# cyu0330/ptbxl-multimodal

Hardware: AMD Instinct MI355X
Metric: ECG windows/s (train step) at 12x1000, batch 256 (higher is better)
Workload: dtype f32; 1 GPU; ECGCNN(5) train step fwd+BCE+bwd+AdamW, 12x1000, fp32, batch 256/GPU, global batch 256; global_batch=256, parallelism=dp1, loop=train_one_epoch, optimizer=FlatAdamW, priming_steps=30

## Files before the change

include/ecg_hip.h:

```cpp
#ifndef ECG_HIP_H
#define ECG_HIP_H

#include <stddef.h>
#include <stdint.h>

#ifdef __cplusplus
extern "C" {
#endif

typedef void *ecg_stream_t;

enum {
    ECG_OK = 0,
    ECG_EINVAL = 1,
    ECG_ELAUNCH = 2,
    ECG_ENODEV = 3
};

int ecg_version(void);
const char *ecg_last_error(void);
int ecg_check_device(void);


int ecg_conv1d_pack_weights(const float *w, float *w_fwd, float *w_bwd,
// ... 6 lines not shown
int ecg_pack_weights_grouped_mixed(const float *const *w, float *const *w_fwd, float *const *w_bwd,
                                   void *const *wb_fwd, void *const *wb_bwd, const int *C_out,
                                   const int *C_in, const int *K, int count, ecg_stream_t stream);

int ecg_conv1d_fwd_stat_partials(int N, int C_in, int C_out, int L, int K, int pad);

int ecg_conv1d_fwd(const float *x, const float *w_fwd, const float *bias, float *y,
                   float *stat_partials, int N, int C_in, int C_out, int L, int K, int pad,
                   ecg_stream_t stream);

int ecg_conv1d_bwd_data(const float *dy, const float *w_bwd, float *dx,
                        int N, int C_in, int C_out, int L, int K, int pad, ecg_stream_t stream);

int ecg_conv1d_dy_row_stride(int N, int C_in, int C_out, int L, int K, int pad, int need_dx);

int ecg_conv1d_multiplies_per_output_pair(int op, int C_in, int C_out, int K, int pad);
int ecg_conv1d_bwd_data_ld(const float *dy, int ldy, const float *w_bwd, float *dx,
                           int N, int C_in, int C_out, int L, int K, int pad, ecg_stream_t stream);
int ecg_conv1d_bwd_weight_bias_ld(const float *dy, int ldy, const float *x, float *dw, float *db,
                                  float *ws, int N, int C_in, int C_out, int L, int K, int pad,
                                  ecg_stream_t stream);

size_t ecg_conv1d_bwd_weight_ws_floats(int N, int C_in, int C_out, int L, int K, int pad);
int ecg_conv1d_bwd_weight_bias(const float *dy, const float *x, float *dw, float *db, float *ws,
                               int N, int C_in, int C_out, int L, int K, int pad,
                               ecg_stream_t stream);

int ecg_conv1d_bf16_supported(int C_in, int C_out, int K, int pad);
size_t ecg_conv1d_bf16_packed_elems(int C_reduce, int C_result, int K);
int ecg_conv1d_pack_weights_bf16(const float *w, void *wb_fwd, void *wb_bwd, int C_out, int C_in,
                                 int K, ecg_stream_t stream);
int ecg_conv1d_fwd_bf16_yh(const void *x, int x_bf16, int ldx, const void *wb_fwd, const float *bias, void *y_bf16,
                           int ldy, float *stat_partials, int N, int C_in, int C_out, int L, int K, int pad,
                           ecg_stream_t stream);
int ecg_conv1d_fwd_bf16_yh_stat_partials(int N, int C_in, int C_out, int L, int K, int pad, int x_bf16, int ldx, int ldy);
int ecg_conv1d_bf16_ring_tile(int N, int C_red, int C_res, int L_out, int K, int pad, int ld_in, int ld_out);
int ecg_bn_stats_relu_pool_fwd_h(const float *stat_partials, int P, long long count, float *running_mean,
                                 float *running_var, long long *num_batches_tracked, float momentum, float eps,
                                 const void *y_bf16, int ldy, const float *gamma, const float *beta, float *mean,
                                 float *invstd, void *p_bf16, int ldp, int N, int C, int L, ecg_stream_t stream);
int ecg_bn_stats_relu_pool_gap_fwd_yh(const float *stat_partials, int P, long long count, float *running_mean,
                                      float *running_var, long long *num_batches_tracked, float momentum, float eps,
                                      const void *y_bf16, int ldy, const float *gamma, const float *beta, float *mean,
                                      float *invstd, float *out, int N, int C, int L, ecg_stream_t stream);
int ecg_bn_relu_pool_bwd_h(const void *y_bf16, int ldyy, const void *dp, int dp_kind, int ldp, const float *gamma,
                           const float *beta, const float *mean, const float *invstd, void *dy_bf16, int ldy,
// ... 159 lines not shown
```

ptbxl-multimodal_amd/csrc/conv1d_api.hip:

```cpp
#include "common.h"

namespace ecg {
int direct_fwd_stat_partials(int N, int Lo);
int direct_fwd(const float *x, const float *wp, const float *bias, float *y, float *partials,
               int N, int Cin, int Cout, int L, int K, int pad, hipStream_t st);
size_t direct_wgrad_ws_floats(int N, int Cin, int Cout, int K);
int direct_wgrad(const float *dy, const float *x, float *dw, float *db, float *ws, int N, int Cin,
                 int Cout, int L, int K, int pad, hipStream_t st);
int pack_weights(const float *w, float *w_fwd, float *w_bwd, int Co, int Ci, int K,
                 hipStream_t st);
int pack_weights_grouped(const float *const *w, float *const *w_fwd, float *const *w_bwd, void *const *wb_fwd,
                         void *const *wb_bwd, const int *Co, const int *Ci, const int *K, int count, hipStream_t st);
bool mfma_fwd_supported(int Cin, int Cout, int K, int pad);
int mfma_fwd_stat_partials(int N, int Cin, int Cout, int Lo);
int mfma_fwd(const float *x, int ldx, const float *wp, const float *bias, float *y, float *partials,
             int N, int Cin, int Cout, int L, int K, int pad, hipStream_t st);
int mfma_fwd_eval_pool(const float *x, const float *wp, const float *bias, const float *gamma,
                       const float *beta, const float *mean, const float *var, float eps, float *p,
                       int N, int Cin, int Cout, int L, int K, int pad, hipStream_t st, int gap);
bool mfma_fwd_eval_gap_supported(int Cin, int Cout, int L, int K, int pad);
bool mfma_wgrad_supported(int Cin, int Cout, int K, int pad);
size_t mfma_wgrad_ws_floats(int N, int Cin, int Cout, int L, int K, int pad);
bool mfma_wgrad_dma_supported(int Cin, int Cout, int K);
int mfma_multiplies_per_pair(int op, int Cin, int Cout, int K, int pad);
int mfma_wgrad(const float *dy, int ldy, const float *x, float *dw, float *db, float *ws, int N,
               int Cin, int Cout, int L, int K, int pad, hipStream_t st);

static int check_conv_shape(int N, int Cin, int Cout, int L, int K, int pad) {
    ECG_REQUIRE(N > 0 && Cin > 0 && Cout > 0 && L > 0, "conv1d: N=%d C_in=%d C_out=%d L=%d must be > 0",
                N, Cin, Cout, L);
    ECG_REQUIRE(K >= 1 && K <= 31, "conv1d: kernel size %d outside [1,31]", K);
    ECG_REQUIRE(pad >= 0 && pad < K, "conv1d: padding %d outside [0,K)", pad);
    ECG_REQUIRE(L + 2 * pad - K + 1 > 0, "conv1d: empty output (L=%d K=%d pad=%d)", L, K, pad);
    ECG_REQUIRE(N <= 65535, "conv1d: N=%d exceeds grid.z limit 65535", N);
    return ECG_OK;
}
}

using namespace ecg;

ECG_API int ecg_conv1d_pack_weights(const float *w, float *w_fwd, float *w_bwd, int C_out,
                                    int C_in, int K, ecg_stream_t stream) {
    ECG_REQUIRE(w && (w_fwd || w_bwd), "pack_weights: null pointer");
    ECG_REQUIRE(C_out > 0 && C_in > 0 && K >= 1 && K <= 31, "pack_weights: bad shape");
    return pack_weights(w, w_fwd, w_bwd, C_out, C_in, K, as_stream(stream));
// ... 63 lines not shown
                                   int C_in, int C_out, int L, int K, int pad, ecg_stream_t stream) {
    int rc = check_conv_shape(N, C_in, C_out, L, K, pad);
    if (rc) return rc;
    ECG_REQUIRE(dy && w_bwd && dx, "conv1d_bwd_data: null pointer");
    const int Lo = L + 2 * pad - K + 1, padb = K - 1 - pad;
    ECG_REQUIRE(ldy >= Lo, "conv1d_bwd_data: dY row stride %d < row length %d", ldy, Lo);
    if (mfma_fwd_supported(C_out, C_in, K, padb))
        return mfma_fwd(dy, ldy, w_bwd, nullptr, dx, nullptr, N, C_out, C_in, Lo, K, padb, as_stream(stream));
    ECG_REQUIRE(ldy == Lo, "conv1d_bwd_data: this shape needs dense dY rows (stride %d != %d); "
                "use the stride ecg_conv1d_dy_row_stride returns", ldy, Lo);
    return direct_fwd(dy, w_bwd, nullptr, dx, nullptr, N, C_out, C_in, Lo, K, padb, as_stream(stream));
}

ECG_API int ecg_conv1d_bwd_data(const float *dy, const float *w_bwd, float *dx, int N, int C_in,
                                int C_out, int L, int K, int pad, ecg_stream_t stream) {
    return ecg_conv1d_bwd_data_ld(dy, L + 2 * pad - K + 1, w_bwd, dx, N, C_in, C_out, L, K, pad, stream);
}

ECG_API size_t ecg_conv1d_bwd_weight_ws_floats(int N, int C_in, int C_out, int L, int K, int pad) {
    if (mfma_wgrad_supported(C_in, C_out, K, pad)) return mfma_wgrad_ws_floats(N, C_in, C_out, L, K, pad);
    return direct_wgrad_ws_floats(N, C_in, C_out, K);
}

ECG_API int ecg_conv1d_bwd_weight_bias_ld(const float *dy, int ldy, const float *x, float *dw,
                                          float *db, float *ws, int N, int C_in, int C_out, int L,
                                          int K, int pad, ecg_stream_t stream) {
    int rc = check_conv_shape(N, C_in, C_out, L, K, pad);
    if (rc) return rc;
    ECG_REQUIRE(dy && x && dw && ws, "conv1d_bwd_weight_bias: null pointer");
    const int Lo = L + 2 * pad - K + 1;
    ECG_REQUIRE(ldy >= Lo, "conv1d_bwd_weight_bias: dY row stride %d < row length %d", ldy, Lo);
    if (mfma_wgrad_supported(C_in, C_out, K, pad))
        return mfma_wgrad(dy, ldy, x, dw, db, ws, N, C_in, C_out, L, K, pad, as_stream(stream));
    ECG_REQUIRE(ldy == Lo, "conv1d_bwd_weight_bias: this shape needs dense dY rows (stride %d != %d); "
                "use the stride ecg_conv1d_dy_row_stride returns", ldy, Lo);
    return direct_wgrad(dy, x, dw, db, ws, N, C_in, C_out, L, K, pad, as_stream(stream));
}

ECG_API int ecg_conv1d_bwd_weight_bias(const float *dy, const float *x, float *dw, float *db,
                                       float *ws, int N, int C_in, int C_out, int L, int K, int pad,
                                       ecg_stream_t stream) {
    return ecg_conv1d_bwd_weight_bias_ld(dy, L + 2 * pad - K + 1, x, dw, db, ws, N, C_in, C_out, L, K,
                                         pad, stream);
}

ECG_API int ecg_conv1d_bn_relu_pool_eval_supported(int C_in, int C_out, int K, int pad) {
// ... 42 lines not shown
```

ptbxl-multimodal_amd/csrc/conv1d_mfma.hip:

```cpp
#include "common.h"
#include <cstdlib>
#include <type_traits>

namespace ecg {

typedef float f32x16 __attribute__((ext_vector_type(16)));
typedef float f32x4 __attribute__((ext_vector_type(4)));

constexpr int kKM = 15;

#ifdef ECG_STAMP
__device__ unsigned long long *g_stamps = nullptr;
#define ECG_STAMP_AT(slot) do { if (g_stamps && threadIdx.x == 0) { \
    g_stamps[(size_t)blockIdx.x * 8 + (slot)] = __builtin_amdgcn_s_memtime(); \
    if ((slot) == 0) g_stamps[(size_t)blockIdx.x * 8 + 7] = __builtin_amdgcn_s_memrealtime(); \
    if ((slot) == 4) g_stamps[(size_t)blockIdx.x * 8 + 6] = __builtin_amdgcn_s_memrealtime(); } } while (0)
#else
#define ECG_STAMP_AT(slot) do { } while (0)
#endif

__device__ __forceinline__ f32x16 mfma32(float a, float b, f32x16 c) {
    return __builtin_amdgcn_mfma_f32_32x32x2f32(a, b, c, 0, 0, 0);
}

__device__ __forceinline__ void glds16(const void *base_in, unsigned voff, unsigned dst) {
    const unsigned long long b = (unsigned long long)base_in;
    const unsigned blo = (unsigned)__builtin_amdgcn_readfirstlane((int)(unsigned)b);
    const unsigned bhi = (unsigned)__builtin_amdgcn_readfirstlane((int)(unsigned)(b >> 32));
    const void *base = (const void *)(((unsigned long long)bhi << 32) | blo);
    unsigned keep;
    asm volatile("s_mov_b32 %0, m0\n\ts_mov_b32 m0, %3\n\ts_nop 0\n\tglobal_load_lds_dwordx4 %1, %2\n\ts_mov_b32 m0, %0"
                 : "=&s"(keep) : "v"(voff), "s"(base), "s"(dst) : "memory");
}

__device__ __forceinline__ void wait_lgkm_f(int n) {
    switch (n) {
        case 1: __builtin_amdgcn_s_waitcnt(0xC17F); break;
        case 2: __builtin_amdgcn_s_waitcnt(0xC27F); break;
        case 3: __builtin_amdgcn_s_waitcnt(0xC37F); break;
        case 4: __builtin_amdgcn_s_waitcnt(0xC47F); break;
        default: break;
    }
}

__device__ __forceinline__ int acc_row(int r, int half) { return (r & 3) + 8 * (r >> 2) + 4 * half; }

enum { EPI_PLAIN = 0, EPI_STATS = 1, EPI_EVAL = 2, EPI_EVAL_GAP = 3 };
#ifndef ECG_FWD_FL
#define ECG_FWD_FL 1
#endif

__device__ __forceinline__ int xcd_chunked(int bid, int nwg) {
    const int q = nwg >> 3, r = nwg & 7, xcd = bid & 7;
    return (xcd < r ? xcd * (q + 1) : r * (q + 1) + (xcd - r) * q) + (bid >> 3);
}
struct EvalEpi { const float *gamma, *beta, *mean, *var; float eps; int gap; };

template <int CO_T, int T_T, int WCO, int WT, int EPI>
__global__ __launch_bounds__(256, 2) void conv1d_mfma_fwd_kernel(
    const float *__restrict__ x, const float *__restrict__ wp, const float *__restrict__ bias,
    float *__restrict__ y, float *__restrict__ partials, int Cin, int Cout, int L, int ldx, int Lo,
    int pad, int P, int tiles_t, EvalEpi ev) {
    constexpr bool STATS = (EPI == EPI_STATS), GAP = (EPI == EPI_EVAL_GAP);
    static_assert(WCO * WT == 4, "4 waves per workgroup");
    constexpr int KK = kKM, CI_C = 4, NST = KK * CI_C / 2;
    constexpr int MC = CO_T / WCO / 32, MT = T_T / WT / 32;
    static_assert(MC >= 1 && MT >= 1, "wave tile must hold at least one 32x32 accumulator");
    constexpr int XS = T_T + 16;
    constexpr int WSZ = KK * CI_C * CO_T;
    constexpr int NDMA = (WSZ + 255) / 256;
    constexpr int WPAD = NDMA * 256;
    constexpr int DPW = (NDMA + 3) / 4;
    constexpr int XEL = CI_C * XS;
    constexpr int XLOADS = (XEL + 255) / 256;
    constexpr int IMG = WPAD + XEL;
    constexpr int REDF = (STATS || GAP) ? 4 * (CO_T / WCO) * 2 : 0;
    static_assert(REDF <= IMG, "stat scratch aliases image 0");
    static_assert(NST >= 2 + DPW + XLOADS, "not enough steps to spread the staging over");
// ... 861 lines not shown
    static_assert(NST % 4 == 0, "whole groups of four steps");
    constexpr int XSPAN = T_T + KK - 1;
    constexpr int XS = ((XSPAN - KK + 31) / 32) * 32 + KK;
    constexpr int NCI = (R_T + KK - 2) / KK + 1;
    constexpr int XEL = NCI * XS, XLOADS = (XEL + 255) / 256;
    constexpr int AEL = M_T * T_T;
    constexpr int NDMA = AEL / 256;
    constexpr int DPW = NDMA / 4;
    constexpr int IMG = ((AEL + XEL + 63) / 64) * 64;
    constexpr int ACCF = MC * MR * 16 * 64;
    static_assert(WK == 1 || WM * WR * ACCF + 4 * 32 <= 2 * IMG, "accumulator exchange must fit the dead images");
    static_assert(XS >= XSPAN, "x row stride too small");
    static_assert(NDMA % 4 == 0, "dY image must split evenly over the four waves");
    static_assert(XLOADS <= 32, "mask bits");
    static_assert(NST >= 2 * XLOADS + DPW, "not enough steps to spread the staging over");

    __shared__ __attribute__((aligned(1024))) float lds[2 * IMG];
    ECG_STAMP_AT(0);

    const int tid = threadIdx.x, lane = tid & 63, wave = tid >> 6;
    const int half = lane >> 5, l31 = lane & 31;
    const int R = Cin * KK;
    const int RT = (R + R_T - 1) / R_T, CT = Cout / M_T;
    const int tile = xcd_chunked(blockIdx.x, gridDim.x);
    const int tile_r = tile % RT, tile_cs = tile / RT;
    const int r0 = tile_r * R_T, co0 = (tile_cs % CT) * M_T, s = tile_cs / CT;
    const int wk = wave % WK, wr = (wave / WK) % WR, wm = wave / (WK * WR);
    const int wm0 = wm * (M_T / WM), wr0 = wr * (R_T / WR), wt0 = wk * TW;
    const int ci_base = r0 / KK;
    const int ntt = (Lo + T_T - 1) / T_T;
    const int it_begin = (int)((long long)N * ntt * s / S), it_end = (int)((long long)N * ntt * (s + 1) / S);

    int xcol[MR];
#pragma unroll
    for (int j = 0; j < MR; ++j) {
        int r = r0 + wr0 + 32 * j + l31;
        if (r >= R) r = R - 1;
        const int ci = r / KK;
        xcol[j] = (ci - ci_base) * XS + (r - ci * KK);
    }

    f32x16 acc[MC][MR], acc2[MC][MR];
    f32x16 zero16;
#pragma unroll
    for (int r = 0; r < 16; ++r) zero16[r] = 0.f;
#pragma unroll
    for (int a = 0; a < MC; ++a)
#pragma unroll
        for (int b = 0; b < MR; ++b) { acc[a][b] = zero16; acc2[a][b] = zero16; }
    float bsum[MC], bsum2[MC];
#pragma unroll
    for (int a = 0; a < MC; ++a) bsum[a] = bsum2[a] = 0.f;
    const bool want_bias = (tile_r == 0) && (wr == 0);

// ... 187 lines not shown
    asm volatile("s_waitcnt vmcnt(0)" ::: "memory");
#endif
    ECG_STAMP_AT(4);
}

template <int M_T, int R_T, int WM, int WR, int FL, int T_T>
__global__ __launch_bounds__(256, 2) void conv1d_mfma_wgrad_ffa_kernel(
    const float *__restrict__ dy, const float *__restrict__ x, float *__restrict__ slab, int N,
    int Cin, int Cout, int L, int Lo, int ldy, int pad, int S) {
    static_assert(WM * WR == 4, "4 waves per workgroup");
    static_assert(kKM == 15, "tap split 8 + 7");
    static_assert(T_T == 64 || T_T == 128, "64 or 128 time steps per stage");
    constexpr int LPR = T_T / 4, RPP = 64 / LPR;
    constexpr int MC = M_T / WM / 32, MR = R_T / WR / 32;
    constexpr int NST = T_T / 4, NGRP = NST / 4;
    constexpr int XS = T_T + 16;
    static_assert(XS % 64 == 16, "x rows 16 banks apart");
    constexpr int NCI = (R_T + 6) / 7 + 1;
    constexpr int XEL = NCI * XS, XLOADS = (XEL + 255) / 256;
    constexpr int AEL = M_T * T_T;
    constexpr int NDMA = AEL / 256;
    constexpr int DPW = NDMA / 4;
    constexpr int IMG = ((AEL + XEL + 63) / 64) * 64;
    constexpr int OPS = 2 * XLOADS + DPW;
    static_assert(NDMA % 4 == 0, "dY image must split evenly over the four waves");
    static_assert(XLOADS <= 32, "mask bits");
    static_assert(2 * IMG * 4 <= 80 * 1024, "two workgroups per CU");

    __shared__ __attribute__((aligned(1024))) float lds[2 * IMG];
    ECG_STAMP_AT(0);

    const int tid = threadIdx.x, lane = tid & 63, wave = tid >> 6;
    const int half = lane >> 5, l31 = lane & 31;
    const int RU = Cin * 8, RV = Cin * 7;
    const int TU = (RU + R_T - 1) / R_T, TV = (RV + R_T - 1) / R_T;
    const int RT = 2 * TU + TV, CT = Cout / M_T;
    const int tile = xcd_chunked(blockIdx.x, gridDim.x);
    const int tile_r = tile % RT, tile_cs = tile / RT;
    const int fam = tile_r < TU ? 0 : (tile_r < TU + TV ? 1 : 2);
    const int tile_rf = tile_r - (fam == 0 ? 0 : (fam == 1 ? TU : TU + TV));
    const int NJ = fam == 1 ? 7 : 8, RF = Cin * NJ, offf = fam == 0 ? 0 : (fam == 1 ? RU : RU + RV);
    const int r0 = tile_rf * R_T, co0 = (tile_cs % CT) * M_T, s = tile_cs / CT;
    const int wr = wave % WR, wm = wave / WR;
    const int wm0 = wm * (M_T / WM), wr0 = wr * (R_T / WR);
    const int ci_base = r0 / NJ;
    const int ntt = (Lo + T_T - 1) / T_T;
    const int it_begin = (int)((long long)N * ntt * s / S), it_end = (int)((long long)N * ntt * (s + 1) / S);

    int xcol[MR];
#pragma unroll
    for (int j = 0; j < MR; ++j) {
        int r = r0 + wr0 + 32 * j + l31;
        if (r >= RF) r = RF - 1;
        const int ci = r / NJ;
        xcol[j] = (ci - ci_base) * XS + 2 * (r - ci * NJ) + 8 * half;
    }

    f32x16 acc[MC][MR], acc2[MC][MR];
    f32x16 zero16;
#pragma unroll
    for (int r = 0; r < 16; ++r) zero16[r] = 0.f;
#pragma unroll
    for (int a = 0; a < MC; ++a)
#pragma unroll
        for (int b = 0; b < MR; ++b) { acc[a][b] = zero16; acc2[a][b] = zero16; }
    float bsum[MC], bsum2[MC];
#pragma unroll
    for (int a = 0; a < MC; ++a) bsum[a] = bsum2[a] = 0.f;
    const bool want_bias = (tile_r == 0) && (wr == 0);

    int doff[DPW];
#pragma unroll
    for (int j = 0; j < DPW; ++j) {
        const int row = (j * 4 + wave) * RPP + lane / LPR;
        doff[j] = row * ldy + (((lane % LPR) ^ (row & 15)) << 2);
    }
    float xreg[XLOADS];
    unsigned xmask = 0, cxmask = 0;
    const int total = it_end - it_begin;

    int sn = it_begin / ntt, stt = it_begin - sn * ntt;
    int dn = sn, dtt = stt;
    auto advance = [&]() { if (++stt == ntt) { stt = 0; ++sn; } };
    const unsigned lds_base = (unsigned)(size_t)(__attribute__((address_space(3))) float *)lds;
    const int wave_u = __builtin_amdgcn_readfirstlane(wave);
    auto dma_a = [&](int j, float *img) {
        const float *base = dy + ((size_t)min(dn, N - 1) * Cout + co0) * ldy + dtt * T_T;
        glds16(base, (unsigned)doff[j] * 4u,
               (unsigned)__builtin_amdgcn_readfirstlane((int)(lds_base + (unsigned)((img - lds) + (j * 4 + wave_u) * 256) * 4u)));
    };
    auto load_x = [&](int j) {
        const float *xn = x + (size_t)min(sn, N - 1) * Cin * L;
        const int e = min(tid + 256 * j, XEL - 1), row = e / XS;
        const int sidx = stt * T_T + (e - row * XS) - pad;
        xreg[j] = xn[min(ci_base + row, Cin - 1) * L + min(max(sidx, 0), L - 1)];
        const unsigned bit = ((sidx >= 0) && (sidx < L)) ? (1u << j) : 0u;
        xmask = (j == 0) ? bit : (xmask | bit);
    };
    auto commit_x = [&](int j, float *img) {
        const int e = tid + 256 * j;
        const unsigned keep = 0u - ((cxmask >> j) & 1u);
        if (256 * (j + 1) <= XEL || e < XEL)
            img[AEL + e] = __uint_as_float(__float_as_uint(xreg[j]) & keep);
    };

    if (total > 0) {
#pragma unroll
        for (int j = 0; j < DPW; ++j) dma_a(j, lds);
#pragma unroll
        for (int j = 0; j < XLOADS; ++j) load_x(j);
        cxmask = xmask;
#pragma unroll
        for (int j = 0; j < XLOADS; ++j) commit_x(j, lds);
        advance();
        dn = sn; dtt = stt;
#pragma unroll
        for (int j = 0; j < XLOADS; ++j) load_x(j);
        advance();
    }
    asm volatile("s_waitcnt vmcnt(0)" ::: "memory");
    __syncthreads();
    ECG_STAMP_AT(1);

    typedef float f32x2t __attribute__((ext_vector_type(2)));
    const int aoff = (wm0 + l31) * T_T, swz = (l31 & 15) << 2;
    auto stage = [&](auto fam_c, int it) {
        constexpr int FAM = decltype(fam_c)::value;
        const float *dys = lds + (it & 1) * IMG, *xs = dys + AEL;
        float *nxt = lds + ((it + 1) & 1) * IMG;
        cxmask = xmask;
        const float *arow = dys + aoff;
        auto lda_lo = [&](int g, f32x4 *lo, float *prev) {
#pragma unroll
            for (int i = 0; i < MC; ++i) {
                const float *rb = arow + 32 * i * T_T;
                const int c0 = 4 * g + 2 * half;
                lo[i] = *reinterpret_cast<const f32x4 *>(rb + ((c0 << 2) ^ swz));
                if (FAM == 1) {
                    const float pv = rb[((max(c0 - 1, 0) << 2) ^ swz) + 3];
                    prev[i] = (g == 0 && half == 0) ? 0.f : pv;
                }
            }
        };
        auto lda_hi = [&](int g, f32x4 *hi) {
#pragma unroll
            for (int i = 0; i < MC; ++i)
                hi[i] = *reinterpret_cast<const f32x4 *>(arow + 32 * i * T_T + (((4 * g + 2 * half + 1) << 2) ^ swz));
        };
        auto ldb = [&](int st, f32x2t *b) {
            const int tp = 16 * (st >> 2) + 2 * (st & 3);
#pragma unroll
            for (int j = 0; j < MR; ++j) b[j] = *reinterpret_cast<const f32x2t *>(xs + xcol[j] + tp);
        };
        f32x4 lo_c[MC], hi_c[MC], lo_n[MC];
        float pv_c[MC], pv_n[MC];
        f32x2t b_c[MR], b_n[MR];
        lda_lo(0, lo_c, pv_c);
        lda_hi(0, hi_c);
        ldb(0, b_c);
#pragma unroll
        for (int st = 0; st < NST; ++st) {
            const int j4 = st & 3;
            ldb(st + 1 < NST ? st + 1 : 0, b_n);
            if (j4 == 2 && (st >> 2) + 1 < NGRP) lda_lo((st >> 2) + 1, lo_n, pv_n);
            if (j4 == 0 && st > 0) lda_hi(st >> 2, hi_c);
#pragma unroll
            for (int o = st * OPS / NST; o < (st + 1) * OPS / NST; ++o) {
                if (o < DPW) dma_a(o, nxt);
                else if (o < DPW + XLOADS) commit_x(o - DPW, nxt);
                else load_x(o - DPW - XLOADS);
            }
            float av[MC], bv[MR];
#pragma unroll
            for (int i = 0; i < MC; ++i) {
                const f32x4 d = j4 < 2 ? lo_c[i] : hi_c[i];
                const float d0 = d[2 * (j4 & 1)], d1 = d[2 * (j4 & 1) + 1];
                const float dp = j4 == 0 ? pv_c[i] : (j4 == 1 ? lo_c[i][1] : (j4 == 2 ? lo_c[i][3] : hi_c[i][1]));
                av[i] = FAM == 0 ? d0 + d1 : (FAM == 1 ? d0 + dp : d1);
            }
#pragma unroll
            for (int j = 0; j < MR; ++j) bv[j] = FAM == 0 ? b_c[j][0] : (FAM == 1 ? b_c[j][1] : b_c[j][0] - b_c[j][1]);
            __builtin_amdgcn_sched_barrier(0);
            if (FAM == 0) {
#pragma unroll
                for (int i = 0; i < MC; ++i) bsum[i] = (FL && st == 0) ? av[i] : bsum[i] + av[i];
            }
#pragma unroll
            for (int i = 0; i < MC; ++i)
#pragma unroll
                for (int j = 0; j < MR; ++j)
                    acc[i][j] = mfma32(av[i], bv[j], (FL && st == 0) ? zero16 : acc[i][j]);
            __builtin_amdgcn_sched_barrier(0);
#pragma unroll
            for (int j = 0; j < MR; ++j) b_c[j] = b_n[j];
// ... 2 lines not shown
                for (int i = 0; i < MC; ++i) { lo_c[i] = lo_n[i]; pv_c[i] = pv_n[i]; }
            }
        }
        if (FAM == 1) {
#pragma unroll
            for (int i = 0; i < MC; ++i) {
                const float dl = arow[32 * i * T_T + (((LPR - 1) << 2) ^ swz) + 3];
                const float a = half ? 0.f : dl;
#pragma unroll
                for (int j = 0; j < MR; ++j)
                    acc[i][j] = mfma32(a, xs[xcol[j] - 8 * half + T_T + 1], acc[i][j]);
            }
        }
        if (FL) {
#pragma unroll
            for (int i = 0; i < MC; ++i)
#pragma unroll
                for (int j = 0; j < MR; ++j) acc2[i][j] += acc[i][j];
            if (FAM == 0) {
#pragma unroll
                for (int i = 0; i < MC; ++i) bsum2[i] += bsum[i];
            }
        }
        dn = sn; dtt = stt;
        advance();
        asm volatile("s_waitcnt vmcnt(%0)" :: "n"(XLOADS) : "memory");
        __syncthreads();
    };
    if (fam == 0) { for (int it = 0; it < total; ++it) { stage(std::integral_constant<int, 0>{}, it); if (it == 0) ECG_STAMP_AT(2); } }
    else if (fam == 1) { for (int it = 0; it < total; ++it) { stage(std::integral_constant<int, 1>{}, it); if (it == 0) ECG_STAMP_AT(2); } }
    else { for (int it = 0; it < total; ++it) { stage(std::integral_constant<int, 2>{}, it); if (it == 0) ECG_STAMP_AT(2); } }
    ECG_STAMP_AT(3);
#ifdef ECG_STAMP
    if (g_stamps && threadIdx.x == 0)
        g_stamps[(size_t)blockIdx.x * 8 + 5] = (unsigned long long)(total & 0xFFFF) |
            ((unsigned long long)__builtin_amdgcn_s_getreg((31 << 11) | 4) << 16) |
            ((unsigned long long)(__builtin_amdgcn_s_getreg((31 << 11) | 20) & 0xF) << 48);
#endif

    if (FL) {
#pragma unroll
        for (int i = 0; i < MC; ++i) {
            bsum[i] = bsum2[i];
#pragma unroll
            for (int j = 0; j < MR; ++j) acc[i][j] = acc2[i][j];
        }
    }
    if (want_bias) {
#pragma unroll
// ... 64 lines not shown
                a[0] += (double)pu[off]; a[1] += (double)pg[off]; a[2] += (double)pv[off]; a[3] += (double)pg[off + g1];
            }
        } else {
            const float *src = slab + (size_t)S * wslab + (i - npair);
            for (int s = w; s < S; s += G) a[0] += (double)src[(size_t)s * Cout];
        }
    }
    if (live) {
        if (i < npair) {
            dw[o] = (float)(a[0] - a[1]);
            if (j < 7) dw[o + 1] = (float)(a[2] + a[3]);
        } else db[i - npair] = (float)a[0];
    }
}

int wgrad_reduce(const float *ws, float *dw, float *db, size_t wslab, int Cout, int S,
                 hipStream_t st);

#ifndef ECG_WG_FL
#define ECG_WG_FL 1
#endif
struct WgCfg { int m_t, r_t, splits; };

#ifndef ECG_WG_SLOTS
#define ECG_WG_SLOTS 512
#endif
#ifndef ECG_WG_RT
#define ECG_WG_RT 0
#endif
#ifndef ECG_WG_TT128
#define ECG_WG_TT128 1
#endif

static WgCfg wgrad_cfg(int N, int Cin, int Cout, int Lo, bool dma, int tt = 64) {
    const int R = Cin * kKM;
    constexpr int slots = ECG_WG_SLOTS, rt128 = ECG_WG_RT;
    WgCfg c;
    const bool wide = dma && !ECG_WG_FL && R % 192 == 0 && (rt128 == 192 || (rt128 == 0 && R % 128 != 0));
    if (Cout % 128 == 0) c = {128, wide ? 192 : 128, 0};
    else if (Cout % 64 == 0) c = {64, 128, 0};
    else c = {32, 192, 0};
    const int tiles = cdiv(R, c.r_t) * (Cout / c.m_t);
    int s = slots / tiles;
    const long long cap = dma ? (long long)N * cdiv(Lo, tt) : N;
    if (s > cap) s = (int)cap;
    if (s < 1) s = 1;
    c.splits = s;
    return c;
}
// ... 20 lines not shown
}

bool mfma_wgrad_supported(int Cin, int Cout, int K, int pad) {
    (void)pad; (void)Cin;
    return K == kKM && Cout % 32 == 0;
}

size_t mfma_wgrad_ws_floats(int N, int Cin, int Cout, int L, int K, int pad) {
    const int Lo = L + 2 * pad - K + 1;
    const WgCfg a = wgrad_cfg(N, Cin, Cout, Lo, false), b = wgrad_cfg(N, Cin, Cout, Lo, true);
    size_t need = (size_t)(a.splits > b.splits ? a.splits : b.splits) * ((size_t)Cout * Cin * K + Cout);
    if (wgrad_ffa_ok(Cin, Cout, true)) {
        const size_t ffa = (size_t)wgrad_ffa_splits(N, Cin, Cout, Lo) * ((size_t)Cout * Cin * 23 + Cout);
        if (ffa > need) need = ffa;
    }
    return need;
}

bool mfma_wgrad_dma_supported(int Cin, int Cout, int K) {
    (void)Cin;
    return K == kKM && Cout % 32 == 0;
}

int mfma_wgrad(const float *dy, int ldy, const float *x, float *dw, float *db, float *ws, int N,
               int Cin, int Cout, int L, int K, int pad, hipStream_t st) {
    const int Lo = L + 2 * pad - K + 1;
    const int R = Cin * K;
    const bool dma = mfma_wgrad_dma_supported(Cin, Cout, K) && ldy % 64 == 0 && ldy >= cdiv(Lo, 64) * 64 &&
                     (reinterpret_cast<uintptr_t>(dy) & 15) == 0;
    const bool tt128 = ECG_WG_TT128 && dma && Cout % 128 != 0 && ldy % 128 == 0 && ldy >= cdiv(Lo, 128) * 128;
    if (wgrad_ffa_ok(Cin, Cout, dma)) {
        const int S = wgrad_ffa_splits(N, Cin, Cout, Lo), m_t = Cout % 128 == 0 ? 128 : 64;
        const int tiles = (2 * cdiv(Cin * 8, 128) + cdiv(Cin * 7, 128)) * (Cout / m_t);
        dim3 fgrid((unsigned)(tiles * S)), fblock(256);
        if (m_t == 128)
            hipLaunchKernelGGL((conv1d_mfma_wgrad_ffa_kernel<128, 128, 2, 2, ECG_WG_FL, 64>), fgrid, fblock, 0, st, dy, x, ws, N, Cin,
                               Cout, L, Lo, ldy, pad, S);
        else
            hipLaunchKernelGGL((conv1d_mfma_wgrad_ffa_kernel<64, 128, 2, 2, ECG_WG_FL, 64>), fgrid, fblock, 0, st, dy, x, ws, N, Cin,
                               Cout, L, Lo, ldy, pad, S);
        int frc = check_launch("conv1d_mfma_wgrad_ffa_kernel");
        if (frc) return frc;
        const size_t nout = (size_t)Cout * Cin * 8 + Cout;
        const dim3 rgrid((unsigned)cdiv(nout, (size_t)64));
        hipLaunchKernelGGL(wgrad_ffa_reduce_kernel, rgrid, dim3(64), 0, st, ws, dw, db, Cin, Cout, S);
        return check_launch("wgrad_ffa_reduce_kernel");
    }
    const WgCfg c = wgrad_cfg(N, Cin, Cout, Lo, dma, tt128 ? 128 : 64);
    dim3 grid((unsigned)(cdiv(R, c.r_t) * (Cout / c.m_t) * c.splits)), block(256);
#define ECG_WG(KERNEL) \
    hipLaunchKernelGGL(KERNEL, grid, block, 0, st, dy, x, ws, N, Cin, Cout, L, Lo, ldy, pad, c.splits)
#if !ECG_WG_FL
    if (dma && c.m_t == 128 && c.r_t == 192) ECG_WG((conv1d_mfma_wgrad_dma_kernel<128, 192, 2, 2, 1, kKM, 0>));
    else
#endif
    if (dma && c.m_t == 128) ECG_WG((conv1d_mfma_wgrad_dma_kernel<128, 128, 2, 2, 1, kKM, ECG_WG_FL>));
    else if (tt128 && c.m_t == 64) ECG_WG((conv1d_mfma_wgrad_dma_kernel<64, 128, 2, 2, 1, kKM, ECG_WG_FL, 128>));
    else if (tt128) ECG_WG((conv1d_mfma_wgrad_dma_kernel<32, 192, 1, 2, 2, kKM, ECG_WG_FL, 128>));
    else if (dma && c.m_t == 64) ECG_WG((conv1d_mfma_wgrad_dma_kernel<64, 128, 2, 2, 1, kKM, ECG_WG_FL>));
    else if (dma) ECG_WG((conv1d_mfma_wgrad_dma_kernel<32, 192, 1, 2, 2, kKM, ECG_WG_FL>));
    else if (c.m_t == 128) ECG_WG((conv1d_mfma_wgrad_kernel<128, 128, 2, 2, 1, 64, kKM, ECG_WG_FL>));
    else if (c.m_t == 64) ECG_WG((conv1d_mfma_wgrad_kernel<64, 128, 2, 2, 1, 64, kKM, ECG_WG_FL>));
    else ECG_WG((conv1d_mfma_wgrad_kernel<32, 192, 1, 2, 2, 128, kKM, ECG_WG_FL>));
#undef ECG_WG
    int rc = check_launch("conv1d_mfma_wgrad_kernel");
    if (rc) return rc;
    return wgrad_reduce(ws, dw, db, (size_t)Cout * R, Cout, c.splits, st);
}

}

#ifdef ECG_STAMP
extern "C" __attribute__((visibility("default"))) int ecg_debug_set_stamp_buffer(unsigned long long *buf) {
    return (int)hipMemcpyToSymbol(HIP_SYMBOL(ecg::g_stamps), &buf, sizeof(buf));
}
#endif
```

ptbxl-multimodal_amd/ecg_hip/_lib.py:

```python
import ctypes
import functools
import os
import threading

import torch

_HERE = os.path.dirname(os.path.abspath(__file__))
LIB_PATH = os.environ.get("ECG_HIP_LIB") or os.path.join(os.path.dirname(_HERE), "lib", "libecg_hip.so")

_vp, _i, _f, _sz, _ll = ctypes.c_void_p, ctypes.c_int, ctypes.c_float, ctypes.c_size_t, ctypes.c_longlong

SIGNATURES = {
    "ecg_version": (_i, []),
    "ecg_last_error": (ctypes.c_char_p, []),
    "ecg_check_device": (_i, []),
    "ecg_conv1d_pack_weights": (_i, [_vp, _vp, _vp, _i, _i, _i, _vp]),
    "ecg_pack_weights_grouped": (_i, [_vp, _vp, _vp, _vp, _vp, _vp, _i, _vp]),
    "ecg_bn_relu_pool_bwd_one_launch_splits": (_i, [_i, _i, _i, _i]),
    "ecg_bn_relu_pool_bwd_one_launch_counter_uints": (_sz, [_i, _i, _i, _i]),
    "ecg_bn_relu_pool_bwd_one_launch": (_i, [_vp] * 7 + [_i] + [_vp] * 3 + [_i] * 6 + [_vp]),
    "ecg_pack_weights_grouped_mixed": (_i, [_vp, _vp, _vp, _vp, _vp, _vp, _vp, _vp, _i, _vp]),
    "ecg_conv1d_fwd_stat_partials": (_i, [_i, _i, _i, _i, _i, _i]),
    "ecg_conv1d_fwd": (_i, [_vp, _vp, _vp, _vp, _vp, _i, _i, _i, _i, _i, _i, _vp]),
    "ecg_conv1d_bwd_data": (_i, [_vp, _vp, _vp, _i, _i, _i, _i, _i, _i, _vp]),
    "ecg_conv1d_bwd_weight_ws_floats": (_sz, [_i, _i, _i, _i, _i, _i]),
    "ecg_conv1d_bwd_weight_bias": (_i, [_vp, _vp, _vp, _vp, _vp, _i, _i, _i, _i, _i, _i, _vp]),
    "ecg_conv1d_dy_row_stride": (_i, [_i] * 7),
    "ecg_conv1d_multiplies_per_output_pair": (_i, [_i] * 5),
    "ecg_conv1d_bwd_data_ld": (_i, [_vp, _i, _vp, _vp, _i, _i, _i, _i, _i, _i, _vp]),
    "ecg_conv1d_bwd_weight_bias_ld": (_i, [_vp, _i, _vp, _vp, _vp, _vp, _i, _i, _i, _i, _i, _i, _vp]),
    "ecg_conv1d_bf16_supported": (_i, [_i, _i, _i, _i]),
    "ecg_conv1d_bf16_packed_elems": (_sz, [_i, _i, _i]),
    "ecg_conv1d_pack_weights_bf16": (_i, [_vp, _vp, _vp, _i, _i, _i, _vp]),
    "ecg_conv1d_fwd_bf16_yh": (_i, [_vp, _i, _i, _vp, _vp, _vp, _i, _vp] + [_i] * 6 + [_vp]),
    "ecg_conv1d_fwd_bf16_yh_stat_partials": (_i, [_i] * 9),
    "ecg_conv1d_bf16_ring_tile": (_i, [_i] * 8),
    "ecg_bn_stats_relu_pool_fwd_h": (_i, [_vp, _i, _ll, _vp, _vp, _vp, _f, _f, _vp, _i, _vp, _vp, _vp, _vp, _vp, _i, _i, _i, _i, _vp]),
    "ecg_bn_relu_pool_bwd_h": (_i, [_vp, _i, _vp, _i, _i] + [_vp] * 5 + [_i] + [_vp] * 3 + [_i] * 4 + [_vp]),
    "ecg_conv1d_bwd_data_bf16hh": (_i, [_vp, _i, _vp, _vp, _i] + [_i] * 6 + [_vp]),
    "ecg_conv1d_bf16_tk_supported": (_i, [_i] * 4),
    "ecg_conv1d_bf16_tk_dy_stride": (_i, [_i]),
    "ecg_conv1d_bwd_weight_bf16_ncl_ws_floats": (_sz, [_i] * 6),
    "ecg_conv1d_bwd_weight_bias_bf16_ncl": (_i, [_vp, _i, _vp, _i, _i, _vp, _vp, _vp] + [_i] * 6 + [_vp]),
    "ecg_bn_stat_partials_count": (_i, [_i, _i, _i]),
    "ecg_bn_stat_partials": (_i, [_vp, _vp, _i, _i, _i, _vp]),
    "ecg_bn_finalize": (_i, [_vp, _i, _ll, _vp, _vp, _vp, _vp, _vp, _i, _f, _f, _vp]),
    "ecg_bn_invstd": (_i, [_vp, _vp, _i, _f, _vp]),
    "ecg_bn_relu_pool_fwd": (_i, [_vp, _vp, _vp, _vp, _vp, _vp, _i, _i, _i, _vp]),
# ... 157 lines not shown
```

Before: 182,000 windows/s.

## Stage wgrad x tile via direct global-to-LDS DMA and add skewed split scheduler

The FFA weight-gradient kernel now loads the x image straight into LDS with masked global_load_lds_dword (on by default), replacing register loads plus masked commits. The DMA issues are spread over the first three quarters of each stage, followed by a full vmcnt wait. A new wgrad_split scheduler can give paired workgroups unequal shares of the time range when skew is nonzero, with a host query API to inspect the split. Skew defaults to zero, so the default path keeps the old even split. The x DMA cuts VGPR use and VALU work, at the cost of exec/m0 juggling and zeroing out-of-range lanes.

Result: no change. 182,900 windows/s, median of 6 (+0.5%).

```diff
diff --git a/include/ecg_hip.h b/include/ecg_hip.h
--- a/include/ecg_hip.h
+++ b/include/ecg_hip.h
@@ -52,6 +52,8 @@
                                   ecg_stream_t stream);
 
 size_t ecg_conv1d_bwd_weight_ws_floats(int N, int C_in, int C_out, int L, int K, int pad);
+int ecg_conv1d_bwd_weight_split(int N, int C_in, int C_out, int L, int K, int pad, int ldy, int skew_permille, int block,
+                                int *grid, int *tile, int *split, int *stages, int *begin, int *end, int *partner);
 int ecg_conv1d_bwd_weight_bias(const float *dy, const float *x, float *dw, float *db, float *ws,
                                int N, int C_in, int C_out, int L, int K, int pad,
                                ecg_stream_t stream);
diff --git a/ptbxl-multimodal_amd/csrc/conv1d_api.hip b/ptbxl-multimodal_amd/csrc/conv1d_api.hip
--- a/ptbxl-multimodal_amd/csrc/conv1d_api.hip
+++ b/ptbxl-multimodal_amd/csrc/conv1d_api.hip
@@ -21,6 +21,7 @@
 bool mfma_fwd_eval_gap_supported(int Cin, int Cout, int L, int K, int pad);
 bool mfma_wgrad_supported(int Cin, int Cout, int K, int pad);
 size_t mfma_wgrad_ws_floats(int N, int Cin, int Cout, int L, int K, int pad);
+int mfma_wgrad_split(int N, int Cin, int Cout, int L, int K, int pad, int ldy, int skew, int block, int *out);
 bool mfma_wgrad_dma_supported(int Cin, int Cout, int K);
 int mfma_multiplies_per_pair(int op, int Cin, int Cout, int K, int pad);
 int mfma_wgrad(const float *dy, int ldy, const float *x, float *dw, float *db, float *ws, int N,
@@ -130,6 +131,23 @@
     return direct_wgrad_ws_floats(N, C_in, C_out, K);
 }
 
+ECG_API int ecg_conv1d_bwd_weight_split(int N, int C_in, int C_out, int L, int K, int pad, int ldy, int skew_permille, int block,
+                                        int *grid, int *tile, int *split, int *stages, int *begin, int *end, int *partner) {
+    int rc = check_conv_shape(N, C_in, C_out, L, K, pad);
+    if (rc) return rc;
+    ECG_REQUIRE(grid && tile && split && stages && begin && end && partner, "conv1d_bwd_weight_split: null pointer");
+    ECG_REQUIRE(mfma_wgrad_supported(C_in, C_out, K, pad), "conv1d_bwd_weight_split: C_out %d, K %d take the direct kernel, "
+                "which has no stage split", C_out, K);
+    ECG_REQUIRE(ldy >= L + 2 * pad - K + 1, "conv1d_bwd_weight_split: dY row stride %d < row length", ldy);
+    ECG_REQUIRE(skew_permille < 1000, "conv1d_bwd_weight_split: skew %d permille (shares are 1 + d and 1 - d, d < 1)", skew_permille);
+    int o[7] = {0, 0, 0, 0, 0, 0, -1};
+    const int bad = mfma_wgrad_split(N, C_in, C_out, L, K, pad, ldy, skew_permille, block, o);
+    *grid = o[0]; *stages = o[3];
+    ECG_REQUIRE(!bad, "conv1d_bwd_weight_split: workgroup %d outside the grid of %d", block, o[0]);
+    *tile = o[1]; *split = o[2]; *begin = o[4]; *end = o[5]; *partner = o[6];
+    return 0;
+}
+
 ECG_API int ecg_conv1d_bwd_weight_bias_ld(const float *dy, int ldy, const float *x, float *dw,
                                           float *db, float *ws, int N, int C_in, int C_out, int L,
                                           int K, int pad, ecg_stream_t stream) {
diff --git a/ptbxl-multimodal_amd/csrc/conv1d_mfma.hip b/ptbxl-multimodal_amd/csrc/conv1d_mfma.hip
--- a/ptbxl-multimodal_amd/csrc/conv1d_mfma.hip
+++ b/ptbxl-multimodal_amd/csrc/conv1d_mfma.hip
@@ -33,6 +33,18 @@
                  : "=&s"(keep) : "v"(voff), "s"(base), "s"(dst) : "memory");
 }
 
+__device__ __forceinline__ void glds4m(const void *base_in, unsigned voff, unsigned dst, unsigned long long lanes) {
+    const unsigned long long b = (unsigned long long)base_in;
+    const unsigned blo = (unsigned)__builtin_amdgcn_readfirstlane((int)(unsigned)b);
+    const unsigned bhi = (unsigned)__builtin_amdgcn_readfirstlane((int)(unsigned)(b >> 32));
+    const void *base = (const void *)(((unsigned long long)bhi << 32) | blo);
+    unsigned keep;
+    unsigned long long ex;
+    asm volatile("s_mov_b32 %0, m0\n\ts_mov_b32 m0, %4\n\ts_mov_b64 %1, exec\n\ts_mov_b64 exec, %5\n\t"
+                 "global_load_lds_dword %2, %3\n\ts_mov_b64 exec, %1\n\ts_mov_b32 m0, %0"
+                 : "=&s"(keep), "=&s"(ex) : "v"(voff), "s"(base), "s"(dst), "s"(lanes) : "memory");
+}
+
 __device__ __forceinline__ void wait_lgkm_f(int n) {
     switch (n) {
         case 1: __builtin_amdgcn_s_waitcnt(0xC17F); break;
@@ -50,10 +62,58 @@
 #define ECG_FWD_FL 1
 #endif
 
-__device__ __forceinline__ int xcd_chunked(int bid, int nwg) {
+__host__ __device__ __forceinline__ int xcd_chunked(int bid, int nwg) {
     const int q = nwg >> 3, r = nwg & 7, xcd = bid & 7;
     return (xcd < r ? xcd * (q + 1) : r * (q + 1) + (xcd - r) * q) + (bid >> 3);
 }
+
+struct WgSplit { int tile_r, cot, s, begin, end; };
+__host__ __device__ inline WgSplit wgrad_split(int bid, int nwg, int RT, int CT, int S, long long total, int dpm, int slots) {
+    WgSplit o;
+    const int T = RT * CT, H = slots / 2;
+    if (dpm <= 0 || nwg > slots || nwg <= H) {
+        const int tile = xcd_chunked(bid, nwg), tcs = tile / RT;
+        o.tile_r = tile % RT; o.cot = tcs % CT; o.s = tcs / CT;
+        o.begin = (int)(total * o.s / S); o.end = (int)(total * (o.s + 1) / S);
+        return o;
+    }
+    const int NP = nwg - H;
+    int Cc = S / 2;
+    if ((long long)Cc * T > NP) Cc = NP / T;
+    const int Lf = S - 2 * Cc, NC = T * Cc, J2 = 2 * (NP - NC);
+    const int hb = bid >= H ? 1 : 0;
+    int q = -1, j = -1;
+    if (hb || bid < NP) {
+        const int pq = xcd_chunked(hb ? bid - H : bid, NP);
+        if (pq < NC) q = pq; else j = 2 * (pq - NC) + hb;
+    } else j = J2 + (bid - NP);
+    const int lin = q >= 0 ? q : j, u = lin / RT;
+    o.tile_r = lin % RT; o.cot = u % CT;
+    const int idx = u / CT;
+    long long before = 0, all = 2000LL * Cc, own = 0;
+    for (int l = 0; l < Lf; ++l) {
+        const int jl = (l * CT + o.cot) * RT + o.tile_r;
+        const int wl = 1000 + (jl < J2 ? ((jl & 1) ? -dpm : dpm) : 0);
+        if (q < 0 && l < idx) before += wl;
+        if (q < 0 && l == idx) own = wl;
+        all += wl;
+    }
+    if (q >= 0) { o.s = 2 * idx + hb; before = 2000LL * idx + (hb ? 1000 + dpm : 0); own = hb ? 1000 - dpm : 1000 + dpm; }
+    else { o.s = 2 * Cc + idx; before += 2000LL * Cc; }
+    o.begin = (int)(total * before / all); o.end = (int)(total * (before + own) / all);
+    return o;
+}
+#ifndef ECG_WG_XDMA
+#define ECG_WG_XDMA 1
+#endif
+#ifndef ECG_WG_SLOTS
+#define ECG_WG_SLOTS 512
+#endif
+#ifndef ECG_WG_SKEW_PERMILLE
+#define ECG_WG_SKEW_PERMILLE 0
+#endif
+constexpr int wg_skew_ffa(int m_t) { return m_t == 128 ? ECG_WG_SKEW_PERMILLE : 0; }
+constexpr int wg_skew_dma(int m_t, int tt) { return m_t == 128 && tt == 64 ? ECG_WG_SKEW_PERMILLE : 0; }
 struct EvalEpi { const float *gamma, *beta, *mean, *var; float eps; int gap; };
 
 template <int CO_T, int T_T, int WCO, int WT, int EPI>
@@ -961,14 +1021,13 @@
     const int half = lane >> 5, l31 = lane & 31;
     const int R = Cin * KK;
     const int RT = (R + R_T - 1) / R_T, CT = Cout / M_T;
-    const int tile = xcd_chunked(blockIdx.x, gridDim.x);
-    const int tile_r = tile % RT, tile_cs = tile / RT;
-    const int r0 = tile_r * R_T, co0 = (tile_cs % CT) * M_T, s = tile_cs / CT;
+    const int ntt = (Lo + T_T - 1) / T_T;
+    const WgSplit sp = wgrad_split(blockIdx.x, gridDim.x, RT, CT, S, (long long)N * ntt, wg_skew_dma(M_T, T_T), ECG_WG_SLOTS);
+    const int tile_r = sp.tile_r, s = sp.s, it_begin = sp.begin, it_end = sp.end;
+    const int r0 = tile_r * R_T, co0 = sp.cot * M_T;
     const int wk = wave % WK, wr = (wave / WK) % WR, wm = wave / (WK * WR);
     const int wm0 = wm * (M_T / WM), wr0 = wr * (R_T / WR), wt0 = wk * TW;
     const int ci_base = r0 / KK;
-    const int ntt = (Lo + T_T - 1) / T_T;
-    const int it_begin = (int)((long long)N * ntt * s / S), it_end = (int)((long long)N * ntt * (s + 1) / S);
 
     int xcol[MR];
 #pragma unroll
@@ -1202,7 +1261,11 @@
     constexpr int NDMA = AEL / 256;
     constexpr int DPW = NDMA / 4;
     constexpr int IMG = ((AEL + XEL + 63) / 64) * 64;
+#if ECG_WG_XDMA
+    constexpr int OPS = DPW + (XEL / 64 + 3) / 4;
+#else
     constexpr int OPS = 2 * XLOADS + DPW;
+#endif
     static_assert(NDMA % 4 == 0, "dY image must split evenly over the four waves");
     static_assert(XLOADS <= 32, "mask bits");
     static_assert(2 * IMG * 4 <= 80 * 1024, "two workgroups per CU");
@@ -1215,17 +1278,16 @@
     const int RU = Cin * 8, RV = Cin * 7;
     const int TU = (RU + R_T - 1) / R_T, TV = (RV + R_T - 1) / R_T;
     const int RT = 2 * TU + TV, CT = Cout / M_T;
-    const int tile = xcd_chunked(blockIdx.x, gridDim.x);
-    const int tile_r = tile % RT, tile_cs = tile / RT;
+    const int ntt = (Lo + T_T - 1) / T_T;
+    const WgSplit sp = wgrad_split(blockIdx.x, gridDim.x, RT, CT, S, (long long)N * ntt, wg_skew_ffa(M_T), ECG_WG_SLOTS);
+    const int tile_r = sp.tile_r, s = sp.s, it_begin = sp.begin, it_end = sp.end;
     const int fam = tile_r < TU ? 0 : (tile_r < TU + TV ? 1 : 2);
     const int tile_rf = tile_r - (fam == 0 ? 0 : (fam == 1 ? TU : TU + TV));
     const int NJ = fam == 1 ? 7 : 8, RF = Cin * NJ, offf = fam == 0 ? 0 : (fam == 1 ? RU : RU + RV);
-    const int r0 = tile_rf * R_T, co0 = (tile_cs % CT) * M_T, s = tile_cs / CT;
+    const int r0 = tile_rf * R_T, co0 = sp.cot * M_T;
     const int wr = wave % WR, wm = wave / WR;
     const int wm0 = wm * (M_T / WM), wr0 = wr * (R_T / WR);
     const int ci_base = r0 / NJ;
-    const int ntt = (Lo + T_T - 1) / T_T;
-    const int it_begin = (int)((long long)N * ntt * s / S), it_end = (int)((long long)N * ntt * (s + 1) / S);
 
     int xcol[MR];
 #pragma unroll
@@ -1255,8 +1317,21 @@
         const int row = (j * 4 + wave) * RPP + lane / LPR;
         doff[j] = row * ldy + (((lane % LPR) ^ (row & 15)) << 2);
     }
+#if ECG_WG_XDMA
+    static_assert(XEL % 64 == 0, "whole 64-dword pieces");
+    constexpr int NPX = XEL / 64, XPW = (NPX + 3) / 4;
+    int xoff[XPW];
+    unsigned xcolp[(XPW + 3) / 4] = {};
+#pragma unroll
+    for (int j = 0; j < XPW; ++j) {
+        const int e = min((j * 4 + wave) * 64 + lane, XEL - 1), row = e / XS, col = e - row * XS;
+        xoff[j] = min(ci_base + row, Cin - 1) * L + col;
+        xcolp[j >> 2] |= (unsigned)col << (8 * (j & 3));
+    }
+#else
     float xreg[XLOADS];
     unsigned xmask = 0, cxmask = 0;
+#endif
     const int total = it_end - it_begin;
 
     int sn = it_begin / ntt, stt = it_begin - sn * ntt;
@@ -1269,6 +1344,22 @@
         glds16(base, (unsigned)doff[j] * 4u,
                (unsigned)__builtin_amdgcn_readfirstlane((int)(lds_base + (unsigned)((img - lds) + (j * 4 + wave_u) * 256) * 4u)));
     };
+#if ECG_WG_XDMA
+    const float *xn = x;
+    int t0p = 0;
+    auto x_stage = [&]() { xn = x + (size_t)min(dn, N - 1) * Cin * L; t0p = dtt * T_T - pad; };
+    auto dma_x = [&](int j, float *img) {
+        if (j * 4 + 3 < NPX || j * 4 + wave_u < NPX) {
+            const int col = (int)((xcolp[j >> 2] >> (8 * (j & 3))) & 255u);
+            const bool in = (unsigned)(t0p + col) < (unsigned)L;
+            const unsigned long long lanes = __builtin_amdgcn_ballot_w64(in);
+            const int e = (j * 4 + wave_u) * 64;
+            glds4m(xn, (unsigned)(xoff[j] + t0p) * 4u,
+                   (unsigned)__builtin_amdgcn_readfirstlane((int)(lds_base + (unsigned)((img - lds) + AEL + e) * 4u)), lanes);
+            if (!in) img[AEL + e + lane] = 0.f;
+        }
+    };
+#else
     auto load_x = [&](int j) {
         const float *xn = x + (size_t)min(sn, N - 1) * Cin * L;
         const int e = min(tid + 256 * j, XEL - 1), row = e / XS;
@@ -1283,10 +1374,18 @@
         if (256 * (j + 1) <= XEL || e < XEL)
             img[AEL + e] = __uint_as_float(__float_as_uint(xreg[j]) & keep);
     };
+#endif
 
     if (total > 0) {
 #pragma unroll
         for (int j = 0; j < DPW; ++j) dma_a(j, lds);
+#if ECG_WG_XDMA
+        x_stage();
+#pragma unroll
+        for (int j = 0; j < XPW; ++j) dma_x(j, lds);
+        advance();
+        dn = sn; dtt = stt;
+#else
 #pragma unroll
         for (int j = 0; j < XLOADS; ++j) load_x(j);
         cxmask = xmask;
@@ -1297,6 +1396,7 @@
 #pragma unroll
         for (int j = 0; j < XLOADS; ++j) load_x(j);
         advance();
+#endif
     }
     asm volatile("s_waitcnt vmcnt(0)" ::: "memory");
     __syncthreads();
@@ -1308,7 +1408,11 @@
         constexpr int FAM = decltype(fam_c)::value;
         const float *dys = lds + (it & 1) * IMG, *xs = dys + AEL;
         float *nxt = lds + ((it + 1) & 1) * IMG;
+#if ECG_WG_XDMA
+        x_stage();
+#else
         cxmask = xmask;
+#endif
         const float *arow = dys + aoff;
         auto lda_lo = [&](int g, f32x4 *lo, float *prev) {
 #pragma unroll
@@ -1344,12 +1448,21 @@
             ldb(st + 1 < NST ? st + 1 : 0, b_n);
             if (j4 == 2 && (st >> 2) + 1 < NGRP) lda_lo((st >> 2) + 1, lo_n, pv_n);
             if (j4 == 0 && st > 0) lda_hi(st >> 2, hi_c);
+#if ECG_WG_XDMA
+            constexpr int SPR = NST * 3 / 4;
+#pragma unroll
+            for (int o = min(st, SPR) * OPS / SPR; o < min(st + 1, SPR) * OPS / SPR; ++o) {
+                if (o < DPW) dma_a(o, nxt);
+                else dma_x(o - DPW, nxt);
+            }
+#else
 #pragma unroll
             for (int o = st * OPS / NST; o < (st + 1) * OPS / NST; ++o) {
                 if (o < DPW) dma_a(o, nxt);
                 else if (o < DPW + XLOADS) commit_x(o - DPW, nxt);
                 else load_x(o - DPW - XLOADS);
             }
+#endif
             float av[MC], bv[MR];
 #pragma unroll
             for (int i = 0; i < MC; ++i) {
@@ -1398,9 +1511,15 @@
                 for (int i = 0; i < MC; ++i) bsum2[i] += bsum[i];
             }
         }
+#if ECG_WG_XDMA
+        advance();
+        dn = sn; dtt = stt;
+        asm volatile("s_waitcnt vmcnt(0)" ::: "memory");
+#else
         dn = sn; dtt = stt;
         advance();
         asm volatile("s_waitcnt vmcnt(%0)" :: "n"(XLOADS) : "memory");
+#endif
         __syncthreads();
     };
     if (fam == 0) { for (int it = 0; it < total; ++it) { stage(std::integral_constant<int, 0>{}, it); if (it == 0) ECG_STAMP_AT(2); } }
@@ -1511,9 +1630,6 @@
 #endif
 struct WgCfg { int m_t, r_t, splits; };
 
-#ifndef ECG_WG_SLOTS
-#define ECG_WG_SLOTS 512
-#endif
 #ifndef ECG_WG_RT
 #define ECG_WG_RT 0
 #endif
@@ -1580,22 +1696,55 @@
     return K == kKM && Cout % 32 == 0;
 }
 
+struct WgPlan { int kind, m_t, r_t, tt, RT, CT, S, dpm; long long total; };
+static WgPlan wgrad_plan(int N, int Cin, int Cout, int Lo, int K, int ldy, bool aligned) {
+    const bool dma = mfma_wgrad_dma_supported(Cin, Cout, K) && ldy % 64 == 0 && ldy >= cdiv(Lo, 64) * 64 && aligned;
+    const bool tt128 = ECG_WG_TT128 && dma && Cout % 128 != 0 && ldy % 128 == 0 && ldy >= cdiv(Lo, 128) * 128;
+    WgPlan p;
+    if (wgrad_ffa_ok(Cin, Cout, dma)) {
+        p.kind = 2; p.m_t = Cout % 128 == 0 ? 128 : 64; p.r_t = 128; p.tt = 64;
+        p.RT = 2 * cdiv(Cin * 8, 128) + cdiv(Cin * 7, 128); p.CT = Cout / p.m_t;
+        p.S = wgrad_ffa_splits(N, Cin, Cout, Lo); p.dpm = wg_skew_ffa(p.m_t);
+        p.total = (long long)N * cdiv(Lo, 64);
+        return p;
+    }
+    const WgCfg c = wgrad_cfg(N, Cin, Cout, Lo, dma, tt128 ? 128 : 64);
+    p.kind = dma ? 1 : 0; p.m_t = c.m_t; p.r_t = c.r_t; p.tt = tt128 ? 128 : 64;
+    p.RT = cdiv(Cin * K, c.r_t); p.CT = Cout / c.m_t; p.S = c.splits;
+    p.dpm = dma ? wg_skew_dma(c.m_t, p.tt) : 0;
+    p.total = dma ? (long long)N * cdiv(Lo, p.tt) : N;
+    return p;
+}
+
+int mfma_wgrad_split(int N, int Cin, int Cout, int L, int K, int pad, int ldy, int skew, int block, int *out) {
+    const int Lo = L + 2 * pad - K + 1;
+    WgPlan p = wgrad_plan(N, Cin, Cout, Lo, K, ldy, true);
+    if (skew >= 0 && p.kind != 0) p.dpm = skew;
+    const int grid = p.RT * p.CT * p.S;
+    out[0] = grid; out[3] = (int)p.total;
+    if (block < 0 || block >= grid) return 1;
+    const WgSplit w = wgrad_split(block, grid, p.RT, p.CT, p.S, p.total, p.dpm, ECG_WG_SLOTS);
+    const int H = ECG_WG_SLOTS / 2;
+    const bool on = p.dpm > 0 && grid <= ECG_WG_SLOTS && grid > H;
+    out[1] = w.cot * p.RT + w.tile_r; out[2] = w.s; out[4] = w.begin; out[5] = w.end;
+    out[6] = !on ? -1 : (block >= H ? block - H : (block + H < grid ? block + H : -1));
+    return 0;
+}
+
 int mfma_wgrad(const float *dy, int ldy, const float *x, float *dw, float *db, float *ws, int N,
                int Cin, int Cout, int L, int K, int pad, hipStream_t st) {
     const int Lo = L + 2 * pad - K + 1;
     const int R = Cin * K;
-    const bool dma = mfma_wgrad_dma_supported(Cin, Cout, K) && ldy % 64 == 0 && ldy >= cdiv(Lo, 64) * 64 &&
-                     (reinterpret_cast<uintptr_t>(dy) & 15) == 0;
-    const bool tt128 = ECG_WG_TT128 && dma && Cout % 128 != 0 && ldy % 128 == 0 && ldy >= cdiv(Lo, 128) * 128;
-    if (wgrad_ffa_ok(Cin, Cout, dma)) {
-        const int S = wgrad_ffa_splits(N, Cin, Cout, Lo), m_t = Cout % 128 == 0 ? 128 : 64;
-        const int tiles = (2 * cdiv(Cin * 8, 128) + cdiv(Cin * 7, 128)) * (Cout / m_t);
-        dim3 fgrid((unsigned)(tiles * S)), fblock(256);
-        if (m_t == 128)
-            hipLaunchKernelGGL((conv1d_mfma_wgrad_ffa_kernel<128, 128, 2, 2, ECG_WG_FL, 64>), fgrid, fblock, 0, st, dy, x, ws, N, Cin,
+    const WgPlan c = wgrad_plan(N, Cin, Cout, Lo, K, ldy, (reinterpret_cast<uintptr_t>(dy) & 15) == 0);
+    const bool dma = c.kind != 0, tt128 = c.tt == 128;
+    dim3 grid((unsigned)(c.RT * c.CT * c.S)), block(256);
+    if (c.kind == 2) {
+        const int S = c.S;
+        if (c.m_t == 128)
+            hipLaunchKernelGGL((conv1d_mfma_wgrad_ffa_kernel<128, 128, 2, 2, ECG_WG_FL, 64>), grid, block, 0, st, dy, x, ws, N, Cin,
                                Cout, L, Lo, ldy, pad, S);
         else
-            hipLaunchKernelGGL((conv1d_mfma_wgrad_ffa_kernel<64, 128, 2, 2, ECG_WG_FL, 64>), fgrid, fblock, 0, st, dy, x, ws, N, Cin,
+            hipLaunchKernelGGL((conv1d_mfma_wgrad_ffa_kernel<64, 128, 2, 2, ECG_WG_FL, 64>), grid, block, 0, st, dy, x, ws, N, Cin,
                                Cout, L, Lo, ldy, pad, S);
         int frc = check_launch("conv1d_mfma_wgrad_ffa_kernel");
         if (frc) return frc;
@@ -1604,10 +1753,8 @@
         hipLaunchKernelGGL(wgrad_ffa_reduce_kernel, rgrid, dim3(64), 0, st, ws, dw, db, Cin, Cout, S);
         return check_launch("wgrad_ffa_reduce_kernel");
     }
-    const WgCfg c = wgrad_cfg(N, Cin, Cout, Lo, dma, tt128 ? 128 : 64);
-    dim3 grid((unsigned)(cdiv(R, c.r_t) * (Cout / c.m_t) * c.splits)), block(256);
 #define ECG_WG(KERNEL) \
-    hipLaunchKernelGGL(KERNEL, grid, block, 0, st, dy, x, ws, N, Cin, Cout, L, Lo, ldy, pad, c.splits)
+    hipLaunchKernelGGL(KERNEL, grid, block, 0, st, dy, x, ws, N, Cin, Cout, L, Lo, ldy, pad, c.S)
 #if !ECG_WG_FL
     if (dma && c.m_t == 128 && c.r_t == 192) ECG_WG((conv1d_mfma_wgrad_dma_kernel<128, 192, 2, 2, 1, kKM, 0>));
     else
@@ -1623,7 +1770,7 @@
 #undef ECG_WG
     int rc = check_launch("conv1d_mfma_wgrad_kernel");
     if (rc) return rc;
-    return wgrad_reduce(ws, dw, db, (size_t)Cout * R, Cout, c.splits, st);
+    return wgrad_reduce(ws, dw, db, (size_t)Cout * R, Cout, c.S, st);
 }
 
 }
diff --git a/ptbxl-multimodal_amd/ecg_hip/_lib.py b/ptbxl-multimodal_amd/ecg_hip/_lib.py
--- a/ptbxl-multimodal_amd/ecg_hip/_lib.py
+++ b/ptbxl-multimodal_amd/ecg_hip/_lib.py
@@ -24,6 +24,7 @@
     "ecg_conv1d_fwd": (_i, [_vp, _vp, _vp, _vp, _vp, _i, _i, _i, _i, _i, _i, _vp]),
     "ecg_conv1d_bwd_data": (_i, [_vp, _vp, _vp, _i, _i, _i, _i, _i, _i, _vp]),
     "ecg_conv1d_bwd_weight_ws_floats": (_sz, [_i, _i, _i, _i, _i, _i]),
+    "ecg_conv1d_bwd_weight_split": (_i, [_i] * 9 + [_vp] * 7),
     "ecg_conv1d_bwd_weight_bias": (_i, [_vp, _vp, _vp, _vp, _vp, _i, _i, _i, _i, _i, _i, _vp]),
     "ecg_conv1d_dy_row_stride": (_i, [_i] * 7),
     "ecg_conv1d_multiplies_per_output_pair": (_i, [_i] * 5),
```
